# nikkolasg/playsnark

Hardware: NVIDIA B200
Metric: g1_msm_points_per_s (higher is better)
Workload: dtype u32

## Files before the change

### playsnark_b200/csrc/curve.cuh

```cuda
#pragma once
#include "field.cuh"

namespace ps {

template <bool INLINE>
struct alignas(16) Fp2T {
  Fp c0, c1;
  PS_DEV static Fp mulp(const Fp& a, const Fp& b) { if (INLINE) return a * b; else return fe_mul_call(a, b); }
  PS_DEV static Fp2T zero() { return Fp2T{Fp::zero(), Fp::zero()}; }
  PS_DEV static Fp2T one() { return Fp2T{Fp::one(), Fp::zero()}; }
  PS_DEV bool is_zero() const { return c0.is_zero() && c1.is_zero(); }
  PS_DEV bool operator==(const Fp2T& b) const { return c0 == b.c0 && c1 == b.c1; }
  PS_DEV bool operator!=(const Fp2T& b) const { return !(*this == b); }
  PS_DEV friend Fp2T operator+(const Fp2T& a, const Fp2T& b) { return Fp2T{a.c0 + b.c0, a.c1 + b.c1}; }
  PS_DEV friend Fp2T operator-(const Fp2T& a, const Fp2T& b) { return Fp2T{a.c0 - b.c0, a.c1 - b.c1}; }
  PS_DEV Fp2T neg() const { return Fp2T{c0.neg(), c1.neg()}; }
  PS_DEV Fp2T dbl() const { return Fp2T{c0.dbl(), c1.dbl()}; }
  PS_DEV friend Fp2T operator*(const Fp2T& a, const Fp2T& b) {
    Fp t0 = mulp(a.c0, b.c0);
    Fp t1 = mulp(a.c1, b.c1);
    Fp t2 = mulp(a.c0 + a.c1, b.c0 + b.c1);
    return Fp2T{t0 - t1, t2 - t0 - t1};
  }
  PS_DEV Fp2T sqr() const {
    Fp s = c0 + c1, d = c0 - c1;
    Fp m = mulp(c0, c1);
    return Fp2T{mulp(s, d), m.dbl()};
  }
};
using Fp2 = Fp2T<false>;
using Fp2I = Fp2T<true>;

PS_DEV Fp2 fp2_inv(const Fp2& a) {
  Fp d = fp_inv(fe_mul_call(a.c0, a.c0) + fe_mul_call(a.c1, a.c1));
  return Fp2{fe_mul_call(a.c0, d), fe_mul_call(a.c1, d).neg()};
}

PS_DEV Fp2 fp2_inv_serial(const Fp2& a) {
  Fp d = fp_inv_serial(fe_mul_call(a.c0, a.c0) + fe_mul_call(a.c1, a.c1));
  return Fp2{fe_mul_call(a.c0, d), fe_mul_call(a.c1, d).neg()};
}

template <class F> struct FieldInv;
template <> struct FieldInv<Fp> {
  PS_DEV static Fp inv(const Fp& a) { return fp_inv(a); }
  PS_DEV static Fp inv_serial(const Fp& a) { return fp_inv_serial(a); }
};
template <> struct FieldInv<Fp2> {
  PS_DEV static Fp2 inv(const Fp2& a) { return fp2_inv(a); }
  PS_DEV static Fp2 inv_serial(const Fp2& a) { return fp2_inv_serial(a); }
};
template <> struct FieldInv<Fp2I> {
  PS_DEV static Fp2I inv(const Fp2I& a) { Fp2 r = fp2_inv(Fp2{a.c0, a.c1}); return Fp2I{r.c0, r.c1}; }
  PS_DEV static Fp2I inv_serial(const Fp2I& a) { Fp2 r = fp2_inv_serial(Fp2{a.c0, a.c1}); return Fp2I{r.c0, r.c1}; }
};

template <class F>
struct alignas(16) Affine {
  F x, y;
  PS_DEV bool is_inf() const { return x.is_zero() && y.is_zero(); }
  PS_DEV static Affine inf() { return Affine{F::zero(), F::zero()}; }
  PS_DEV Affine neg() const { return Affine{x, y.neg()}; }
};

template <class F>
struct alignas(16) XYZZ {
  F x, y, zz, zzz;
  PS_DEV bool is_inf() const { return zz.is_zero(); }
  PS_DEV static XYZZ inf() { return XYZZ{F::zero(), F::zero(), F::zero(), F::zero()}; }
  PS_DEV static XYZZ from_affine(const Affine<F>& p) {
    if (p.is_inf()) return inf();
    return XYZZ{p.x, p.y, F::one(), F::one()};
  }
  PS_DEV XYZZ neg() const { return XYZZ{x, y.neg(), zz, zzz}; }
};

PS_DEV Fp mul_sub_pair(const Fp& a, const Fp& b, const Fp& c, const Fp& d) {
#ifndef PS_NO_LAZY_Y3
  return mul2_lazy(a, b, neg_lazy(c), d);
#else
  return a * b - c * d;
#endif
}
template <bool I>
PS_DEV Fp2T<I> mul_sub_pair(const Fp2T<I>& a, const Fp2T<I>& b, const Fp2T<I>& c, const Fp2T<I>& d) { return a * b - c * d; }

template <class F>
PS_DEV XYZZ<F> xyzz_dbl_affine(const Affine<F>& p) {
  if (p.is_inf() || p.y.is_zero()) return XYZZ<F>::inf();
  F U = p.y.dbl();
  F V = U.sqr();
  F W = U * V;
  F S = p.x * V;
  F X2 = p.x.sqr();
  F M = X2.dbl() + X2;
  F X3 = M.sqr() - S.dbl();
  F Y3 = mul_sub_pair(M, S - X3, W, p.y);
  return XYZZ<F>{X3, Y3, V, W};
}

template <class F>
PS_DEV XYZZ<F> xyzz_dbl(const XYZZ<F>& p) {
  if (p.is_inf() || p.y.is_zero()) return XYZZ<F>::inf();
  F U = p.y.dbl();
  F V = U.sqr();
  F W = U * V;
  F S = p.x * V;
  F X2 = p.x.sqr();
  F M = X2.dbl() + X2;
  F X3 = M.sqr() - S.dbl();
  F Y3 = mul_sub_pair(M, S - X3, W, p.y);
  return XYZZ<F>{X3, Y3, V * p.zz, W * p.zzz};
}

template <class F> PS_NOINLINE XYZZ<F> xyzz_dbl_c(const XYZZ<F>& p);
template <class F> PS_NOINLINE XYZZ<F> xyzz_dbl_affine_c(const Affine<F>& p);

template <class F>
PS_DEV void xyzz_madd(XYZZ<F>& acc, const Affine<F>& q) {
  if (q.is_inf()) return;
  if (acc.is_inf()) { acc = XYZZ<F>{q.x, q.y, F::one(), F::one()}; return; }
  F U2 = q.x * acc.zz;
  F S2 = q.y * acc.zzz;
  F Pd = U2 - acc.x;
  F Rd = S2 - acc.y;
  if (Pd.is_zero()) {
    if (Rd.is_zero()) acc = xyzz_dbl_affine_c(q); else acc = XYZZ<F>::inf();
    return;
  }
  F PP = Pd.sqr();
  F PPP = Pd * PP;
  F Q = acc.x * PP;
  F X3 = Rd.sqr() - PPP - Q.dbl();
  F Y3 = mul_sub_pair(Rd, Q - X3, acc.y, PPP);
  acc.x = X3;
  acc.y = Y3;
  acc.zz = acc.zz * PP;
  acc.zzz = acc.zzz * PPP;
}

template <class F>
PS_DEV void xyzz_add(XYZZ<F>& acc, const XYZZ<F>& q) {
  if (q.is_inf()) return;
  if (acc.is_inf()) { acc = q; return; }
  F U1 = acc.x * q.zz;
  F U2 = q.x * acc.zz;
  F S1 = acc.y * q.zzz;
  F S2 = q.y * acc.zzz;
  F Pd = U2 - U1;
  F Rd = S2 - S1;
  if (Pd.is_zero()) {
    if (Rd.is_zero()) acc = xyzz_dbl_c(acc); else acc = XYZZ<F>::inf();
    return;
  }
  F PP = Pd.sqr();
  F PPP = Pd * PP;
  F Q = U1 * PP;
  F X3 = Rd.sqr() - PPP - Q.dbl();
  F Y3 = mul_sub_pair(Rd, Q - X3, S1, PPP);
  acc.x = X3;
  acc.y = Y3;
  acc.zz = acc.zz * q.zz * PP;
  acc.zzz = acc.zzz * q.zzz * PPP;
}

template <class F> PS_NOINLINE XYZZ<F> xyzz_dbl_c(const XYZZ<F>& p) { return xyzz_dbl(p); }
template <class F> PS_NOINLINE XYZZ<F> xyzz_dbl_affine_c(const Affine<F>& p) { return xyzz_dbl_affine(p); }
template <class F> PS_NOINLINE void xyzz_add_c(XYZZ<F>& acc, const XYZZ<F>& q) { xyzz_add(acc, q); }
template <class F> PS_NOINLINE void xyzz_madd_c(XYZZ<F>& acc, const Affine<F>& q) { xyzz_madd(acc, q); }

template <class F>
PS_DEV Affine<F> xyzz_to_affine(const XYZZ<F>& p) {
  if (p.is_inf()) return Affine<F>::inf();
  F zzz_inv = FieldInv<F>::inv(p.zzz);
  F t = zzz_inv * p.zz;
  F zz_inv = t.sqr();
  return Affine<F>{p.x * zz_inv, p.y * zzz_inv};
}

template <class F>
PS_DEV XYZZ<F> xyzz_scalar_mul(const XYZZ<F>& p, const uint32_t* k, int nlimbs) {
  XYZZ<F> acc = XYZZ<F>::inf();
  for (int i = nlimbs - 1; i >= 0; i--) {
    uint32_t w = k[i];
#pragma unroll 1
    for (int b = 31; b >= 0; b--) {
      acc = xyzz_dbl_c(acc);
      if ((w >> b) & 1) xyzz_add_c(acc, p);
    }
  }
  return acc;
}

template <class F> PS_NOINLINE Affine<F> xyzz_to_affine_c(const XYZZ<F>& p) { return xyzz_to_affine(p); }
template <class F>
PS_NOINLINE Affine<F> xyzz_to_affine_serial(const XYZZ<F>& p) {
  if (p.is_inf()) return Affine<F>::inf();
  F zzz_inv = FieldInv<F>::inv_serial(p.zzz);
  F t = zzz_inv * p.zz;
  F zz_inv = t.sqr();
  return Affine<F>{p.x * zz_inv, p.y * zzz_inv};
}

using G1Affine = Affine<Fp>;
using G2Affine = Affine<Fp2>;
using G1XYZZ = XYZZ<Fp>;
using G2XYZZ = XYZZ<Fp2>;

}
```

### playsnark_b200/csrc/msm.cuh

```cuda
#pragma once
#include "group_ops.cuh"
#include "team.cuh"

namespace ps {

PS_DEV int msm_seg_of(const MsmPlan& p, uint32_t i) {
  int k = 0;
  while (k + 1 < p.nseg && i >= p.seg[k + 1].start) k++;
  return k;
}

struct MsmSrc {
  const uint32_t* scalars;
  uint32_t idx, b0, pt, nbase;
  int mont;
};
PS_DEV MsmSrc msm_source(const MsmPlan& p, uint32_t i) {
  MsmSrc s;
  if (p.row_len) {
    const uint32_t set = i / p.row_len;
    s.scalars = p.seg[0].scalars; s.idx = i; s.mont = (int)p.seg[0].mont;
    s.b0 = set * (uint32_t)p.S * p.D; s.nbase = p.nbase[0]; s.pt = p.toff[0] + p.seg[0].first + (i - set * p.row_len);
  } else {
    const MsmSeg sg = p.seg[msm_seg_of(p, i)];
    s.scalars = sg.scalars; s.idx = i - sg.start; s.mont = (int)sg.mont;
    s.b0 = sg.set * (uint32_t)p.S * p.D; s.nbase = p.nbase[sg.set]; s.pt = p.toff[sg.set] + sg.first + s.idx;
  }
  return s;
}

PS_DEV void msm_load_scalar(const uint32_t* scalars, uint32_t i, int mont, uint32_t k[8], bool& neg) {
  Fr x;
#pragma unroll
  for (int j = 0; j < 8; j++) x.v[j] = scalars[(size_t)i * 8 + j];
  if (mont) x = x.from_mont();
  uint32_t t = ptx_sub_cc(FrParams::HALF(0), x.v[0]);
#pragma unroll
  for (int j = 1; j < 8; j++) t = ptx_subc_cc(FrParams::HALF(j), x.v[j]);
  uint32_t borrow = ptx_subc(0, 0);
  neg = borrow != 0;
  if (neg) {
    uint32_t m[8];
    m[0] = ptx_sub_cc(FrParams::MOD(0), x.v[0]);
#pragma unroll
    for (int j = 1; j < 8; j++) m[j] = ptx_subc_cc(FrParams::MOD(j), x.v[j]);
#pragma unroll
    for (int j = 0; j < 8; j++) x.v[j] = m[j];
  }
#pragma unroll
  for (int j = 0; j < 8; j++) k[j] = x.v[j];
}

PS_DEV uint32_t msm_take_bits(uint32_t k[8], int c) {
  uint32_t v = k[0] & ((1u << c) - 1);
#pragma unroll
  for (int j = 0; j < 7; j++) k[j] = (k[j] >> c) | (k[j + 1] << (32 - c));
  k[7] >>= c;
  return v;
}

PS_DEV bool msm_next_digit(uint32_t k[8], int c, uint32_t& carry, uint32_t& mag, bool& dneg) {
  uint32_t v = msm_take_bits(k, c) + carry;
  uint32_t half = 1u << (c - 1);
  if (v > half) { mag = (1u << c) - v; dneg = true; carry = 1; }
  else { mag = v; dneg = false; carry = 0; }
  return mag != 0;
}

struct MsmCountK {
  static constexpr int BLOCK = 256;
  PS_DEV static void run(uint32_t i, MsmPlan p, uint32_t* count, uint32_t* ranks) {
    const MsmSrc src = msm_source(p, i);
    uint32_t k[8]; bool neg;
    msm_load_scalar(src.scalars, src.idx, src.mont, k, neg);
    uint32_t carry = 0;
    for (int w = 0; w < p.W; w++) {
      uint32_t mag; bool dneg;
      uint32_t rank = 0xFFFFFFFFu;
      if (msm_next_digit(k, p.c, carry, mag, dneg)) {
        uint32_t b = src.b0 + (uint32_t)(w / p.T) * p.D + (mag - 1);
        rank = ps_atomic_add(count + b, 1u);
      }
      ranks[(size_t)w * p.total + i] = rank;
    }
  }
};

struct MsmScatterK {
  static constexpr int BLOCK = 256;
  PS_DEV static void run(uint32_t i, MsmPlan p, const uint32_t* off, const uint32_t* ranks, uint32_t* ent) {
    const MsmSrc src = msm_source(p, i);
    uint32_t k[8]; bool neg;
    msm_load_scalar(src.scalars, src.idx, src.mont, k, neg);
    uint32_t carry = 0;
    for (int w = 0; w < p.W; w++) {
      uint32_t mag; bool dneg;
      if (msm_next_digit(k, p.c, carry, mag, dneg)) {
        uint32_t b = src.b0 + (uint32_t)(w / p.T) * p.D + (mag - 1);
        uint32_t pos = off[b] + ranks[(size_t)w * p.total + i];
        uint32_t idx = (uint32_t)(w % p.T) * src.nbase + src.pt;
        ent[pos] = idx | ((neg != dneg) ? 0x80000000u : 0u);
      }
    }
  }
};

PS_DEV uint32_t msm_find_bucket(const uint32_t* off, uint32_t nb, uint32_t pos) {
  uint32_t lo = 0, hi = nb;
  while (hi - lo > 1) {
    uint32_t mid = lo + (hi - lo) / 2;
    if (off[mid] <= pos) lo = mid; else hi = mid;
  }
  return lo;
}

template <class F>
PS_DEV Affine<F> msm_load_point(const Affine<F>* tab, uint32_t e) {
  Affine<F> p = tab[e & 0x7FFFFFFFu];
  if (e >> 31) p.y = p.y.neg();
  return p;
}

#ifndef PS_G1_MINB
#define PS_G1_MINB 3
#endif
#ifndef PS_G2_MINB
#define PS_G2_MINB 2
#endif
#ifndef PS_ACC_BLOCK
#define PS_ACC_BLOCK 128
#endif
template <class F>
struct MsmAccumK {
  static constexpr int BLOCK = PS_ACC_BLOCK;
  static constexpr int MIN_BLOCKS = sizeof(F) == sizeof(Fp) ? PS_G1_MINB : PS_G2_MINB;
  using Self = MsmAccumK<F>;
  PS_DEV static void run(uint32_t tid, uint32_t nb, uint32_t L, const Affine<F>* tab, const uint32_t* ent,
                         const uint32_t* off, XYZZ<F>* buckets, XYZZ<F>* slot_pt, int32_t* slot_bid,
                         uint8_t* slot_fl) {
    const uint32_t M = off[nb];
    const uint32_t head = 2 * tid, tail = 2 * tid + 1;
    slot_bid[head] = -1; slot_bid[tail] = -1;
    uint64_t p0 = (uint64_t)tid * L;
    if (p0 >= M) return;
    uint32_t cur = (uint32_t)p0;
    uint32_t end = (M - cur > L) ? cur + L : M;
    uint32_t b = msm_find_bucket(off, nb, cur);
    bool head_open = off[b] < cur;
    uint32_t bend = off[b + 1];
    XYZZ<F> acc = XYZZ<F>::inf();
    for (; cur < end; cur++) {
      if (cur == bend) {
        flush(b, acc, head_open, true, head, tail, buckets, slot_pt, slot_bid, slot_fl);
        acc = XYZZ<F>::inf();
        head_open = false;
        b++;
        while (off[b + 1] <= cur) b++;
        bend = off[b + 1];
      }
      xyzz_madd(acc, msm_load_point(tab, ent[cur]));
    }
    flush(b, acc, head_open, bend <= end, head, tail, buckets, slot_pt, slot_bid, slot_fl);
  }
  PS_DEV static void flush(uint32_t b, const XYZZ<F>& acc, bool head_open, bool closed, uint32_t head, uint32_t tail,
                           XYZZ<F>* buckets, XYZZ<F>* slot_pt, int32_t* slot_bid, uint8_t* slot_fl) {
    if (closed && !head_open) {
      buckets[b] = acc;
    } else {
      uint32_t s = head_open ? head : tail;
      slot_pt[s] = acc;
      slot_bid[s] = (int32_t)b;
      slot_fl[s] = (uint8_t)((head_open ? 1 : 0) | (closed ? 0 : 2));
    }
  }
};

template <bool T> struct Coop;
template <> struct Coop<false> {
  static constexpr uint32_t LANES = 1;
  PS_DEV explicit Coop(uint32_t&) {}
  template <class F> PS_DEV void add(XYZZ<F>& acc, const XYZZ<F>& q) const { xyzz_add_c(acc, q); }
  template <class F> PS_DEV void dbl(XYZZ<F>& p) const { p = xyzz_dbl_c(p); }
  PS_DEV bool writer() const { return true; }
  PS_DEV bool idle() const { return false; }
  PS_DEV void sync() const {}
};
template <> struct Coop<true> {
  static constexpr uint32_t LANES = TEAM;
  TeamCtx tc;
  PS_DEV explicit Coop(uint32_t& tid) : tc(TeamCtx::of(tid)) { tid >>= 2; }
  template <class F> PS_DEV void add(XYZZ<F>& acc, const XYZZ<F>& q) const { xyzz_add_t(acc, q, tc); }
  template <class F> PS_DEV void dbl(XYZZ<F>& p) const { xyzz_dbl_t(p, tc); }
  PS_DEV bool writer() const { return tc.tl == 0; }
  PS_DEV bool idle() const {
#ifdef __CUDA_ARCH__
    return false;
#else
    return tc.tl != 0;
#endif
  }
  PS_DEV void sync() const { tc.sync(); }
};

template <class F, bool T>
struct MsmRunMergeK {
  static constexpr int BLOCK = 128;
  static constexpr uint32_t RUN_MAX = 32;
  PS_DEV static void run(uint32_t t, uint32_t n_chunks, XYZZ<F>* buckets, XYZZ<F>* slot_pt, int32_t* slot_bid,
                         const uint8_t* slot_fl) {
    Coop<T> co(t);
    if (co.idle()) return;
    const uint32_t a = 2 * t + 1;
    int32_t bid = slot_bid[a];
    if (bid < 0 || slot_fl[a] != 2) return;
    uint32_t len = 0;
    for (uint32_t j = 1; j <= RUN_MAX && t + j < n_chunks; j++) {
      uint32_t h = 2 * (t + j);
      if (slot_bid[h] != bid) return;
      if (slot_fl[h] == 1) { len = j; break; }
    }
    if (!len) return;
    XYZZ<F> acc = slot_pt[a];
    for (uint32_t j = 1; j <= len; j++) co.add(acc, slot_pt[2 * (t + j)]);
    co.sync();
    if (!co.writer()) return;
    buckets[bid] = acc;
    slot_bid[a] = -1;
    for (uint32_t j = 1; j <= len; j++) slot_bid[2 * (t + j)] = -1;
  }
};

template <class F, bool T>
struct MsmCombineK {
  static constexpr int BLOCK = 128;
  PS_DEV static void flush(int32_t bid, const XYZZ<F>& acc, bool cl, bool cr, int final_pass, uint32_t tid,
                           XYZZ<F>* buckets, XYZZ<F>* out_pt, int32_t* out_bid, uint8_t* out_fl) {
    if (bid < 0) return;
    if (final_pass || (!cl && !cr)) { buckets[bid] = acc; return; }
    uint32_t s = cl ? 2 * tid : 2 * tid + 1;
    out_pt[s] = acc; out_bid[s] = bid; out_fl[s] = (uint8_t)((cl ? 1 : 0) | (cr ? 2 : 0));
  }
  PS_DEV static void run(uint32_t tid, uint32_t n_in, uint32_t f, const XYZZ<F>* in_pt, const int32_t* in_bid,
                         const uint8_t* in_fl, XYZZ<F>* buckets, XYZZ<F>* out_pt, int32_t* out_bid,
                         uint8_t* out_fl, int final_pass) {
    Coop<T> co(tid);
    if (co.idle()) return;
    const bool wr = co.writer();
    if (wr) { out_bid[2 * tid] = -1; out_bid[2 * tid + 1] = -1; }
    int32_t cur = -1; bool cl = false, cr = false;
    XYZZ<F> acc = XYZZ<F>::inf();
    for (uint32_t i = 0; i < f; i++) {
      uint64_t j = (uint64_t)tid * f + i;
      if (j >= n_in) break;
      int32_t bid = in_bid[j];
      if (bid < 0) continue;
      uint8_t fl = in_fl[j];
      if (bid != cur) {
        if (wr) flush(cur, acc, cl, cr, final_pass, tid, buckets, out_pt, out_bid, out_fl);
        cur = bid; acc = in_pt[j]; cl = fl & 1; cr = (fl & 2) != 0;
      } else {
        co.add(acc, in_pt[j]); cr = (fl & 2) != 0;
      }
    }
    if (wr) flush(cur, acc, cl, cr, final_pass, tid, buckets, out_pt, out_bid, out_fl);
  }
};

template <class F, bool T>
struct MsmReduceFirstK {
  static constexpr int BLOCK = 128;
  PS_DEV static void run(uint32_t tid, uint32_t D, uint32_t G, uint32_t g, const XYZZ<F>* buckets, XYZZ<F>* acc_out,
                         XYZZ<F>* run_out) {
    Coop<T> co(tid);
    if (co.idle()) return;
    uint32_t s = tid / G, j = tid % G;
    const XYZZ<F>* B = buckets + (size_t)s * D + (size_t)j * g;
    XYZZ<F> rr = XYZZ<F>::inf(), ww = XYZZ<F>::inf();
    for (uint32_t i = g; i-- > 0;) {
      co.add(rr, B[i]);
      co.add(ww, rr);
    }
    if (co.writer()) { acc_out[tid] = ww; run_out[tid] = rr; }
  }
};

template <class F, bool T>
struct MsmReduceK {
  static constexpr int BLOCK = 64;
  PS_DEV static void run(uint32_t tid, uint32_t n_in, uint32_t n_out, uint32_t f, int log_len, const XYZZ<F>* acc_in,
                         const XYZZ<F>* run_in, XYZZ<F>* acc_out, XYZZ<F>* run_out) {
    Coop<T> co(tid);
    if (co.idle()) return;
    uint32_t s = tid / n_out, j = tid % n_out;
    const XYZZ<F>* A = acc_in + (size_t)s * n_in + (size_t)j * f;
    const XYZZ<F>* R = run_in + (size_t)s * n_in + (size_t)j * f;
    XYZZ<F> asum = XYZZ<F>::inf(), rr = XYZZ<F>::inf(), ww = XYZZ<F>::inf();
    for (uint32_t i = f; i-- > 0;) {
      if ((size_t)j * f + i >= n_in) continue;
      co.add(asum, A[i]);
      co.add(rr, R[i]);
      if (i > 0) co.add(ww, rr);
    }
    for (int d = 0; d < log_len; d++) co.dbl(ww);
    co.add(asum, ww);
    if (co.writer()) { acc_out[tid] = asum; run_out[tid] = rr; }
  }
};

template <class F, bool T>
struct MsmBitGatherK {
  static constexpr int BLOCK = 64;
  PS_DEV static void run(uint32_t tid, uint32_t G, int g, const XYZZ<F>* acc, const XYZZ<F>* run, XYZZ<F>* Y) {
    Coop<T> co(tid);
    if (co.idle()) return;
    const uint32_t half = G / 2;
    uint32_t s = tid / ((uint32_t)(g + 1) * half), rem = tid % ((uint32_t)(g + 1) * half);
    uint32_t r = rem / half, i = rem % half;
    XYZZ<F> y;
    if (r == 0) {
      y = acc[(size_t)s * G + 2 * i];
      co.add(y, acc[(size_t)s * G + 2 * i + 1]);
    } else {
      uint32_t k = r - 1;
// ... 386 lines not shown
```

### playsnark_b200/csrc/field.cuh

```cuda
#pragma once
#include <cstdint>
#include "constants.cuh"

namespace ps {

#ifdef __CUDACC__
#define PS_NOINLINE __host__ __device__ __noinline__
#define PS_DEV __host__ __device__ __forceinline__
#else
#define PS_NOINLINE
#define PS_DEV inline
#endif

#ifdef __CUDA_ARCH__
PS_DEV uint32_t ptx_add_cc(uint32_t a, uint32_t b) { uint32_t r; asm volatile("add.cc.u32 %0,%1,%2;" : "=r"(r) : "r"(a), "r"(b)); return r; }
PS_DEV uint32_t ptx_addc_cc(uint32_t a, uint32_t b) { uint32_t r; asm volatile("addc.cc.u32 %0,%1,%2;" : "=r"(r) : "r"(a), "r"(b)); return r; }
PS_DEV uint32_t ptx_addc(uint32_t a, uint32_t b) { uint32_t r; asm volatile("addc.u32 %0,%1,%2;" : "=r"(r) : "r"(a), "r"(b)); return r; }
PS_DEV uint32_t ptx_sub_cc(uint32_t a, uint32_t b) { uint32_t r; asm volatile("sub.cc.u32 %0,%1,%2;" : "=r"(r) : "r"(a), "r"(b)); return r; }
PS_DEV uint32_t ptx_subc_cc(uint32_t a, uint32_t b) { uint32_t r; asm volatile("subc.cc.u32 %0,%1,%2;" : "=r"(r) : "r"(a), "r"(b)); return r; }
PS_DEV uint32_t ptx_subc(uint32_t a, uint32_t b) { uint32_t r; asm volatile("subc.u32 %0,%1,%2;" : "=r"(r) : "r"(a), "r"(b)); return r; }
PS_DEV void ptx_mad_wide_cc(uint32_t& lo, uint32_t& hi, uint32_t a, uint32_t b) {
  asm volatile("mad.lo.cc.u32 %0,%2,%3,%0; madc.hi.cc.u32 %1,%2,%3,%1;" : "+r"(lo), "+r"(hi) : "r"(a), "r"(b)); }
PS_DEV void ptx_madc_wide_cc(uint32_t& lo, uint32_t& hi, uint32_t a, uint32_t b) {
  asm volatile("madc.lo.cc.u32 %0,%2,%3,%0; madc.hi.cc.u32 %1,%2,%3,%1;" : "+r"(lo), "+r"(hi) : "r"(a), "r"(b)); }
PS_DEV void ptx_mul_wide(uint32_t& lo, uint32_t& hi, uint32_t a, uint32_t b) {
  asm volatile("mul.lo.u32 %0,%2,%3; mul.hi.u32 %1,%2,%3;" : "=r"(lo), "=r"(hi) : "r"(a), "r"(b)); }
#else
inline uint32_t& host_cc() { static thread_local uint32_t cc = 0; return cc; }
inline uint32_t ptx_add_cc(uint32_t a, uint32_t b) { uint64_t t = (uint64_t)a + b; host_cc() = (uint32_t)(t >> 32); return (uint32_t)t; }
inline uint32_t ptx_addc_cc(uint32_t a, uint32_t b) { uint64_t t = (uint64_t)a + b + host_cc(); host_cc() = (uint32_t)(t >> 32); return (uint32_t)t; }
inline uint32_t ptx_addc(uint32_t a, uint32_t b) { return a + b + host_cc(); }
inline uint32_t ptx_sub_cc(uint32_t a, uint32_t b) { uint64_t t = (uint64_t)a - b; host_cc() = (uint32_t)(t >> 63); return (uint32_t)t; }
inline uint32_t ptx_subc_cc(uint32_t a, uint32_t b) { uint64_t t = (uint64_t)a - b - host_cc(); host_cc() = (uint32_t)(t >> 63); return (uint32_t)t; }
inline uint32_t ptx_subc(uint32_t a, uint32_t b) { return a - b - host_cc(); }
inline void ptx_mad_wide_cc(uint32_t& lo, uint32_t& hi, uint32_t a, uint32_t b) {
  unsigned __int128 t = (unsigned __int128)a * b + (((uint64_t)hi << 32) | lo);
  lo = (uint32_t)t; hi = (uint32_t)(t >> 32); host_cc() = (uint32_t)(t >> 64); }
inline void ptx_madc_wide_cc(uint32_t& lo, uint32_t& hi, uint32_t a, uint32_t b) {
  unsigned __int128 t = (unsigned __int128)a * b + (((uint64_t)hi << 32) | lo) + host_cc();
  lo = (uint32_t)t; hi = (uint32_t)(t >> 32); host_cc() = (uint32_t)(t >> 64); }
inline void ptx_mul_wide(uint32_t& lo, uint32_t& hi, uint32_t a, uint32_t b) {
  uint64_t t = (uint64_t)a * b; lo = (uint32_t)t; hi = (uint32_t)(t >> 32); }
#endif

template <int N>
PS_DEV void mul_chain(uint32_t* acc, const uint32_t* a, uint32_t b) {
#pragma unroll
  for (int j = 0; j < N; j += 2) ptx_mul_wide(acc[j], acc[j + 1], a[j], b);
}

template <int N, bool CARRY_IN>
PS_DEV void mad_chain(uint32_t* acc, const uint32_t* a, uint32_t b) {
  if (CARRY_IN) ptx_madc_wide_cc(acc[0], acc[1], a[0], b);
  else ptx_mad_wide_cc(acc[0], acc[1], a[0], b);
#pragma unroll
  for (int j = 2; j < N; j += 2) ptx_madc_wide_cc(acc[j], acc[j + 1], a[j], b);
}

template <class P, int OFF>
PS_DEV void mad_chain_mod(uint32_t* acc, uint32_t b) {
  constexpr int N = P::N;
  ptx_mad_wide_cc(acc[0], acc[1], P::MOD(OFF), b);
#pragma unroll
  for (int j = 2; j < N; j += 2) ptx_madc_wide_cc(acc[j], acc[j + 1], P::MOD(OFF + j), b);
}

template <class P> struct Fe;
template <class P> PS_NOINLINE Fe<P> fe_mul_call(const Fe<P>& a, const Fe<P>& b);

template <class P>
struct alignas(16) Fe {
  static constexpr int N = P::N;
  using Params = P;
  uint32_t v[P::N];

  PS_DEV static Fe zero() { Fe r;
#pragma unroll
    for (int i = 0; i < N; i++) r.v[i] = 0;
    return r; }
  PS_DEV static Fe one() { Fe r;
#pragma unroll
    for (int i = 0; i < N; i++) r.v[i] = P::ONE(i);
    return r; }
  template <uint32_t (*LIMB)(int)>
  PS_DEV static Fe from_const() { Fe r;
#pragma unroll
    for (int i = 0; i < N; i++) r.v[i] = LIMB(i);
    return r; }

  PS_DEV bool is_zero() const { uint32_t o = 0;
#pragma unroll
    for (int i = 0; i < N; i++) o |= v[i];
    return o == 0; }
  PS_DEV bool operator==(const Fe& b) const { uint32_t o = 0;
#pragma unroll
    for (int i = 0; i < N; i++) o |= v[i] ^ b.v[i];
    return o == 0; }
  PS_DEV bool operator!=(const Fe& b) const { return !(*this == b); }

  PS_DEV static void final_sub(Fe& a, uint32_t top) {
    uint32_t t[N];
    t[0] = ptx_sub_cc(a.v[0], P::MOD(0));
#pragma unroll
    for (int i = 1; i < N; i++) t[i] = ptx_subc_cc(a.v[i], P::MOD(i));
    uint32_t borrow = ptx_subc(top, 0);
#pragma unroll
    for (int i = 0; i < N; i++) a.v[i] = borrow ? a.v[i] : t[i];
  }

  PS_DEV friend Fe operator+(const Fe& a, const Fe& b) {
    Fe r;
    r.v[0] = ptx_add_cc(a.v[0], b.v[0]);
#pragma unroll
    for (int i = 1; i < N; i++) r.v[i] = ptx_addc_cc(a.v[i], b.v[i]);
    uint32_t top = ptx_addc(0, 0);
    final_sub(r, top);
    return r;
  }
  PS_DEV friend Fe operator-(const Fe& a, const Fe& b) {
    Fe r;
    r.v[0] = ptx_sub_cc(a.v[0], b.v[0]);
#pragma unroll
    for (int i = 1; i < N; i++) r.v[i] = ptx_subc_cc(a.v[i], b.v[i]);
    uint32_t borrow = ptx_subc(0, 0);
    uint32_t t[N];
#pragma unroll
    for (int i = 0; i < N; i++) t[i] = P::MOD(i) & borrow;
    r.v[0] = ptx_add_cc(r.v[0], t[0]);
#pragma unroll
    for (int i = 1; i < N - 1; i++) r.v[i] = ptx_addc_cc(r.v[i], t[i]);
    r.v[N - 1] = ptx_addc(r.v[N - 1], t[N - 1]);
    return r;
  }
  PS_DEV Fe neg() const { return is_zero() ? *this : (Fe::zero() - *this); }
  PS_DEV Fe dbl() const { return *this + *this; }

  PS_DEV friend Fe operator*(const Fe& a, const Fe& b) {
    uint32_t X[N], Y[N];
    uint32_t pend;
    {
      const uint32_t bi = b.v[0];
      mul_chain<N>(X, a.v, bi);
      mul_chain<N>(Y, a.v + 1, bi);
      const uint32_t m = X[0] * P::INV;
      mad_chain_mod<P, 0>(X, m);
      uint32_t cx = ptx_addc(0, 0);
      mad_chain_mod<P, 1>(Y, m);
      pend = X[1];
#pragma unroll
      for (int k = 0; k < N - 2; k++) X[k] = X[k + 2];
      X[N - 2] = cx; X[N - 1] = 0;
    }
#pragma unroll
    for (int i = 1; i < N; i++) {
      const uint32_t bi = b.v[i];
      uint32_t* A = (i & 1) ? Y : X;
      uint32_t* S = (i & 1) ? X : Y;
      A[0] = ptx_add_cc(A[0], pend);
      mad_chain<N, true>(S, a.v + 1, bi);
      mad_chain<N, false>(A, a.v, bi);
      uint32_t cx = ptx_addc(0, 0);
      const uint32_t m = A[0] * P::INV;
      mad_chain_mod<P, 0>(A, m);
      cx = ptx_addc(cx, 0);
      mad_chain_mod<P, 1>(S, m);
      pend = A[1];
#pragma unroll
      for (int k = 0; k < N - 2; k++) A[k] = A[k + 2];
      A[N - 2] = cx; A[N - 1] = 0;
    }
    uint32_t* A = (N & 1) ? Y : X;
    uint32_t* S = (N & 1) ? X : Y;
    Fe r;
    r.v[0] = ptx_add_cc(A[0], pend);
#pragma unroll
    for (int k = 1; k < N; k++) r.v[k] = ptx_addc_cc(A[k], S[k - 1]);
    uint32_t top = ptx_addc(S[N - 1], 0);
    final_sub(r, top);
    return r;
  }
  PS_DEV Fe sqr() const { return (*this) * (*this); }


  PS_DEV Fe to_mont() const { return fe_mul_call(*this, from_const<P::R2>()); }
  PS_DEV Fe from_mont() const { Fe o = zero(); o.v[0] = 1; return fe_mul_call(*this, o); }

  PS_NOINLINE Fe pow(const uint32_t* e, int nlimbs) const {
    Fe acc = one();
    bool started = false;
    for (int i = nlimbs - 1; i >= 0; i--) {
      uint32_t w = e[i];
#pragma unroll 1
      for (int b = 31; b >= 0; b--) {
        if (started) acc = acc * acc;
        if ((w >> b) & 1) {
          if (started) acc = acc * (*this); else { acc = *this; started = true; }
        }
      }
    }
    return acc;
  }
};

template <class P, int OFF>
PS_DEV void madc_chain_mod(uint32_t* acc, uint32_t b) {
  constexpr int N = P::N;
#pragma unroll
  for (int j = 0; j < N; j += 2) ptx_madc_wide_cc(acc[j], acc[j + 1], P::MOD(OFF + j), b);
}

template <class P, bool DUAL>
PS_DEV void wide_rows(uint32_t* E, uint32_t* O, const Fe<P>& a, const Fe<P>& b, const Fe<P>& c, const Fe<P>& d) {
  constexpr int N = P::N;
#pragma unroll
  for (int k = 0; k < 2 * N + 2; k++) { E[k] = 0; O[k] = 0; }
  mul_chain<N>(E, a.v, b.v[0]);
  mul_chain<N>(O + 1, a.v + 1, b.v[0]);
  if (DUAL) {
    mad_chain<N, false>(E, c.v, d.v[0]);
    E[N] = ptx_addc(E[N], 0);
    mad_chain<N, false>(O + 1, c.v + 1, d.v[0]);
    O[N + 1] = ptx_addc(O[N + 1], 0);
  }
#pragma unroll
  for (int i = 1; i < N; i++) {
    uint32_t* ge = (i & 1) ? O : E;
    uint32_t* go = (i & 1) ? E : O;
    mad_chain<N, false>(ge + i, a.v, b.v[i]);
    ge[i + N] = ptx_addc(ge[i + N], 0);
    mad_chain<N, false>(go + i + 1, a.v + 1, b.v[i]);
    go[i + 1 + N] = ptx_addc(go[i + 1 + N], 0);
    if (DUAL) {
      mad_chain<N, false>(ge + i, c.v, d.v[i]);
      ge[i + N] = ptx_addc(ge[i + N], 0);
      mad_chain<N, false>(go + i + 1, c.v + 1, d.v[i]);
      go[i + 1 + N] = ptx_addc(go[i + 1 + N], 0);
    }
  }
}
template <int N>
PS_DEV void wide_merge(uint32_t* T, const uint32_t* E, const uint32_t* O) {
  T[0] = E[0];
  T[1] = ptx_add_cc(E[1], O[1]);
#pragma unroll
  for (int k = 2; k < 2 * N - 1; k++) T[k] = ptx_addc_cc(E[k], O[k]);
  T[2 * N - 1] = ptx_addc(E[2 * N - 1], O[2 * N - 1]);
}
template <class P>
PS_DEV void mul_wide(uint32_t* T, const Fe<P>& a, const Fe<P>& b) {
  constexpr int N = P::N;
  uint32_t E[2 * N + 2], O[2 * N + 2];
  wide_rows<P, false>(E, O, a, b, a, b);
  wide_merge<N>(T, E, O);
}
template <class P>
PS_DEV Fe<P> redc_wide(const uint32_t* T);
template <class P>
PS_DEV void mul2_wide(uint32_t* T, const Fe<P>& a, const Fe<P>& b, const Fe<P>& c, const Fe<P>& d) {
  constexpr int N = P::N;
  uint32_t E[2 * N + 2], O[2 * N + 2];
  wide_rows<P, true>(E, O, a, b, c, d);
  wide_merge<N>(T, E, O);
}
template <class P>
PS_DEV Fe<P> mul2_lazy(const Fe<P>& a, const Fe<P>& b, const Fe<P>& c, const Fe<P>& d) {
  uint32_t T[2 * P::N];
  mul2_wide(T, a, b, c, d);
  return redc_wide<P>(T);
}
template <class P>
PS_DEV Fe<P> neg_lazy(const Fe<P>& a) {
  constexpr int N = P::N;
  Fe<P> r;
  r.v[0] = ptx_sub_cc(P::MOD(0), a.v[0]);
#pragma unroll
  for (int k = 1; k < N - 1; k++) r.v[k] = ptx_subc_cc(P::MOD(k), a.v[k]);
  r.v[N - 1] = ptx_subc(P::MOD(N - 1), a.v[N - 1]);
  return r;
}

template <class P>
PS_DEV Fe<P> redc_wide(const uint32_t* T) {
  constexpr int N = P::N;
  uint32_t X[N], Y[N];
  uint32_t pend;
#pragma unroll
  for (int k = 0; k < N; k++) { X[k] = T[k]; Y[k] = 0; }
  {
    const uint32_t m = X[0] * P::INV;
    mad_chain_mod<P, 0>(X, m);
    uint32_t cx = ptx_addc(0, 0);
    mad_chain_mod<P, 1>(Y, m);
    pend = X[1];
#pragma unroll
    for (int k = 0; k < N - 2; k++) X[k] = X[k + 2];
    X[N - 2] = cx; X[N - 1] = 0;
  }
#pragma unroll
  for (int i = 1; i < N; i++) {
    uint32_t* A = (i & 1) ? Y : X;
    uint32_t* S = (i & 1) ? X : Y;
    const uint32_t m = (A[0] + pend) * P::INV;
    A[0] = ptx_add_cc(A[0], pend);
    madc_chain_mod<P, 1>(S, m);
    mad_chain_mod<P, 0>(A, m);
    uint32_t cx = ptx_addc(0, 0);
    pend = A[1];
#pragma unroll
    for (int k = 0; k < N - 2; k++) A[k] = A[k + 2];
    A[N - 2] = cx; A[N - 1] = 0;
  }
  uint32_t* A = (N & 1) ? Y : X;
  uint32_t* S = (N & 1) ? X : Y;
  Fe<P> r;
  r.v[0] = ptx_add_cc(A[0], pend);
#pragma unroll
  for (int k = 1; k < N; k++) r.v[k] = ptx_addc_cc(A[k], S[k - 1]);
  uint32_t top = ptx_addc(S[N - 1], 0);
  r.v[0] = ptx_add_cc(r.v[0], T[N]);
#pragma unroll
  for (int k = 1; k < N; k++) r.v[k] = ptx_addc_cc(r.v[k], T[N + k]);
  top = ptx_addc(top, 0);
  Fe<P>::final_sub(r, top);
  return r;
}

using Fp = Fe<FpParams>;
using Fr = Fe<FrParams>;

template <class P>
PS_DEV Fe<P> fe_ld(const Fe<P>* p) {
#ifdef __CUDA_ARCH__
  Fe<P> r;
  const uint4* q = reinterpret_cast<const uint4*>(p);
#pragma unroll
  for (int i = 0; i < P::N / 4; i++) {
    uint4 t = __ldg(q + i);
    r.v[4 * i] = t.x; r.v[4 * i + 1] = t.y; r.v[4 * i + 2] = t.z; r.v[4 * i + 3] = t.w;
  }
  return r;
#else
  return *p;
#endif
}

template <class P>
PS_NOINLINE Fe<P> fe_mul_call(const Fe<P>& a, const Fe<P>& b) { return a * b; }

}

namespace ps {
#ifdef __CUDA_ARCH__
#define PS_CEXP(name) name
#else
#define PS_CEXP(name) host_##name()
inline const uint32_t* host_c_FP_MOD_M2() { static uint32_t t[12]; for (int i = 0; i < 12; i++) t[i] = FpParams::MOD_M2(i); return t; }
inline const uint32_t* host_c_FP_SQRT_EXP() { static uint32_t t[12]; for (int i = 0; i < 12; i++) t[i] = FpParams::SQRT_EXP(i); return t; }
inline const uint32_t* host_c_FP_P_M3_D4() { static uint32_t t[12]; for (int i = 0; i < 12; i++) t[i] = FpParams::P_M3_D4(i); return t; }
inline const uint32_t* host_c_FP_P_M1_D2() { static uint32_t t[12]; for (int i = 0; i < 12; i++) t[i] = FpParams::P_M1_D2(i); return t; }
inline const uint32_t* host_c_FR_MOD_M2() { static uint32_t t[8]; for (int i = 0; i < 8; i++) t[i] = FrParams::MOD_M2(i); return t; }
#endif
template <class P>
PS_NOINLINE Fe<P> fe_inv_gcd(const Fe<P>& a) {
  constexpr int N = P::N;
  if (a.is_zero()) return a;
  uint32_t u[N], v[N], x1[N], x2[N];
#pragma unroll
  for (int i = 0; i < N; i++) { u[i] = a.v[i]; v[i] = P::MOD(i); x1[i] = 0; x2[i] = 0; }
  x1[0] = 1;
  auto halve = [](uint32_t* y, uint32_t* x) {
    constexpr int N = P::N;
#pragma unroll
    for (int i = 0; i < N - 1; i++) y[i] = (y[i] >> 1) | (y[i + 1] << 31);
    y[N - 1] >>= 1;
    uint32_t top = 0;
    if (x[0] & 1) {
      x[0] = ptx_add_cc(x[0], P::MOD(0));
#pragma unroll
      for (int i = 1; i < N; i++) x[i] = ptx_addc_cc(x[i], P::MOD(i));
      top = ptx_addc(0, 0);
    }
#pragma unroll
    for (int i = 0; i < N - 1; i++) x[i] = (x[i] >> 1) | (x[i + 1] << 31);
    x[N - 1] = (x[N - 1] >> 1) | (top << 31);
  };
  auto reduce = [](uint32_t* y, const uint32_t* z, uint32_t* x, const uint32_t* w) {
    constexpr int N = P::N;
    y[0] = ptx_sub_cc(y[0], z[0]);
#pragma unroll
    for (int i = 1; i < N - 1; i++) y[i] = ptx_subc_cc(y[i], z[i]);
    y[N - 1] = ptx_subc(y[N - 1], z[N - 1]);
    x[0] = ptx_sub_cc(x[0], w[0]);
#pragma unroll
    for (int i = 1; i < N; i++) x[i] = ptx_subc_cc(x[i], w[i]);
    uint32_t borrow = ptx_subc(0, 0);
    if (borrow) {
      x[0] = ptx_add_cc(x[0], P::MOD(0));
#pragma unroll
      for (int i = 1; i < N - 1; i++) x[i] = ptx_addc_cc(x[i], P::MOD(i));
      x[N - 1] = ptx_addc(x[N - 1], P::MOD(N - 1));
    }
  };
  auto is_one = [](const uint32_t* y) {
    constexpr int N = P::N;
    uint32_t o = y[0] ^ 1u;
#pragma unroll
    for (int i = 1; i < N; i++) o |= y[i];
    return o == 0;
  };
  auto geq = [](const uint32_t* y, const uint32_t* z) {
    constexpr int N = P::N;
    (void)ptx_sub_cc(y[0], z[0]);
#pragma unroll
    for (int i = 1; i < N; i++) (void)ptx_subc_cc(y[i], z[i]);
    return ptx_subc(0, 0) == 0;
  };
#pragma unroll 1
  for (int guard = 0; guard < 4 * 32 * N; guard++) {
    if (is_one(u) || is_one(v)) break;
#pragma unroll 1
    while ((u[0] & 1) == 0) halve(u, x1);
#pragma unroll 1
    while ((v[0] & 1) == 0) halve(v, x2);
    if (geq(u, v)) reduce(u, v, x1, x2); else reduce(v, u, x2, x1);
  }
  Fe<P> y;
  const bool from_u = is_one(u);
#pragma unroll
  for (int i = 0; i < N; i++) y.v[i] = from_u ? x1[i] : x2[i];
  const Fe<P> r2 = Fe<P>::template from_const<P::R2>();
  return y * (r2 * r2);
}
PS_DEV Fp fp_inv(const Fp& a) { return a.pow(PS_CEXP(c_FP_MOD_M2), 12); }
PS_DEV Fr fr_inv(const Fr& a) { return a.pow(PS_CEXP(c_FR_MOD_M2), 8); }
PS_DEV Fp fp_inv_serial(const Fp& a) { return fe_inv_gcd(a); }
PS_DEV Fr fr_inv_serial(const Fr& a) { return fe_inv_gcd(a); }
PS_DEV Fp fp_sqrt_candidate(const Fp& a) { return a.pow(PS_CEXP(c_FP_SQRT_EXP), 12); }
}
```

Measured before the change: 193.0 million.

## Keep G1 bucket accumulator in shared memory and raise G1 min blocks

The G1 bucket-accumulation kernel now keeps its XYZZ accumulator in a strided shared-memory slot per thread instead of in registers. A new slot-based mixed-add routine reads and writes the coordinates through load/store helpers, reordered so fewer field elements are live at once. With fewer live registers, the launch-bounds min-blocks for G1 goes from 3 to 4 to raise occupancy. The cost is extra shared-memory traffic on every add, about 24 KB of shared memory per block, and a pointer offset derived from the top limb's high bits that assumes values are fully reduced.

```diff
diff --git a/playsnark_b200/csrc/curve.cuh b/playsnark_b200/csrc/curve.cuh
--- a/playsnark_b200/csrc/curve.cuh
+++ b/playsnark_b200/csrc/curve.cuh
@@ -139,6 +139,39 @@
   acc.zzz = acc.zzz * PPP;
 }
 
+template <class F, class S>
+PS_DEV void xyzz_madd_slot(S& acc, const Affine<F>& q) {
+  if (q.is_inf()) return;
+  F U2 = acc.ld(2);
+  if (U2.is_zero()) { acc.st(0, q.x); acc.st(1, q.y); acc.st(2, F::one()); acc.st(3, F::one()); return; }
+  U2 = q.x * U2;
+  F S2 = q.y * acc.ld(3);
+  F Pd = U2 - acc.ld(0);
+  F Rd = S2 - acc.ld(1);
+  if (Pd.is_zero()) {
+    if (!Rd.is_zero() || q.y.is_zero()) { acc.st(0, F::zero()); acc.st(1, F::zero()); acc.st(2, F::zero()); acc.st(3, F::zero()); return; }
+    const F U = q.y.dbl();
+    const F X2 = q.x.sqr();
+    acc.st(1, X2.dbl() + X2);
+    acc.st(2, U.sqr());
+    acc.st(3, U * acc.ld(2));
+    acc.st(0, q.x * acc.ld(2));
+    const F M = acc.ld(1), Sx = acc.ld(0);
+    const F X3 = M.sqr() - Sx.dbl();
+    acc.st(0, X3);
+    acc.st(1, mul_sub_pair(M, Sx - X3, acc.ld(3), q.y));
+    return;
+  }
+  F PP = Pd.sqr();
+  acc.st(2, acc.ld(2) * PP);
+  F PPP = Pd * PP;
+  acc.st(3, acc.ld(3) * PPP);
+  F Q = acc.ld(0) * PP;
+  F X3 = Rd.sqr() - PPP - Q.dbl();
+  acc.st(0, X3);
+  acc.st(1, mul_sub_pair(Rd, Q - X3, acc.ld(1), PPP));
+}
+
 template <class F>
 PS_DEV void xyzz_add(XYZZ<F>& acc, const XYZZ<F>& q) {
   if (q.is_inf()) return;
diff --git a/playsnark_b200/csrc/msm.cuh b/playsnark_b200/csrc/msm.cuh
--- a/playsnark_b200/csrc/msm.cuh
+++ b/playsnark_b200/csrc/msm.cuh
@@ -122,7 +122,7 @@
 }
 
 #ifndef PS_G1_MINB
-#define PS_G1_MINB 3
+#define PS_G1_MINB 4
 #endif
 #ifndef PS_G2_MINB
 #define PS_G2_MINB 2
@@ -130,6 +130,48 @@
 #ifndef PS_ACC_BLOCK
 #define PS_ACC_BLOCK 128
 #endif
+
+template <class F>
+struct AccInRegs {
+  XYZZ<F> v;
+  PS_DEV void reset() { v = XYZZ<F>::inf(); }
+  PS_DEV void madd(const Affine<F>& q) { xyzz_madd(v, q); }
+  PS_DEV XYZZ<F> get() const { return v; }
+};
+struct AccInSmemG1 {
+  static constexpr int BLOCK = PS_ACC_BLOCK;
+#ifdef __CUDA_ARCH__
+  uint4* p;
+  PS_DEV AccInSmemG1() {
+    __shared__ uint4 sh[4 * 3 * BLOCK];
+    p = sh + threadIdx.x;
+  }
+  PS_DEV Fp ld(int k) const {
+    Fp r;
+#pragma unroll
+    for (int i = 0; i < 3; i++) {
+      const uint4 t = p[(3 * k + i) * BLOCK];
+      r.v[4 * i] = t.x; r.v[4 * i + 1] = t.y; r.v[4 * i + 2] = t.z; r.v[4 * i + 3] = t.w;
+    }
+    return r;
+  }
+  PS_DEV void st(int k, const Fp& a) {
+#pragma unroll
+    for (int i = 0; i < 3; i++) p[(3 * k + i) * BLOCK] = make_uint4(a.v[4 * i], a.v[4 * i + 1], a.v[4 * i + 2], a.v[4 * i + 3]);
+    p += a.v[11] >> 29;
+  }
+#else
+  Fp v[4];
+  PS_DEV Fp ld(int k) const { return v[k]; }
+  PS_DEV void st(int k, const Fp& a) { v[k] = a; }
+#endif
+  PS_DEV void reset() { st(0, Fp::zero()); st(1, Fp::zero()); st(2, Fp::zero()); st(3, Fp::zero()); }
+  PS_DEV void madd(const Affine<Fp>& q) { xyzz_madd_slot(*this, q); }
+  PS_DEV XYZZ<Fp> get() const { return XYZZ<Fp>{ld(0), ld(1), ld(2), ld(3)}; }
+};
+template <class F> struct AccOf { using T = AccInRegs<F>; };
+template <> struct AccOf<Fp> { using T = AccInSmemG1; };
+
 template <class F>
 struct MsmAccumK {
   static constexpr int BLOCK = PS_ACC_BLOCK;
@@ -148,19 +190,20 @@
     uint32_t b = msm_find_bucket(off, nb, cur);
     bool head_open = off[b] < cur;
     uint32_t bend = off[b + 1];
-    XYZZ<F> acc = XYZZ<F>::inf();
+    typename AccOf<F>::T acc;
+    acc.reset();
     for (; cur < end; cur++) {
       if (cur == bend) {
-        flush(b, acc, head_open, true, head, tail, buckets, slot_pt, slot_bid, slot_fl);
-        acc = XYZZ<F>::inf();
+        flush(b, acc.get(), head_open, true, head, tail, buckets, slot_pt, slot_bid, slot_fl);
+        acc.reset();
         head_open = false;
         b++;
         while (off[b + 1] <= cur) b++;
         bend = off[b + 1];
       }
-      xyzz_madd(acc, msm_load_point(tab, ent[cur]));
-    }
-    flush(b, acc, head_open, bend <= end, head, tail, buckets, slot_pt, slot_bid, slot_fl);
+      acc.madd(msm_load_point(tab, ent[cur]));
+    }
+    flush(b, acc.get(), head_open, bend <= end, head, tail, buckets, slot_pt, slot_bid, slot_fl);
   }
   PS_DEV static void flush(uint32_t b, const XYZZ<F>& acc, bool head_open, bool closed, uint32_t head, uint32_t tail,
                            XYZZ<F>* buckets, XYZZ<F>* slot_pt, int32_t* slot_bid, uint8_t* slot_fl) {
```

After: 194.4 million (median of 6 runs). About the same (+0.7%).

## Use lazy-reduced Montgomery arithmetic in G1 bucket accumulation madd

Applied to the files above, without the earlier changes.

Adds a bound-tracked lazy field type (values kept below 2p) and a variant of the Montgomery multiply and double-product reduction that skips the final conditional subtraction. The G1 bucket accumulation loop now uses a mixed add over these lazily reduced coordinates, with cheaper subtraction, zero tests modulo p, and canonicalisation only when a bucket is flushed. This removes a final_sub per multiply on the hot path, in exchange for extra zero-check comparisons and reliance on the compile-time bound asserts being correct for the BLS12-381 modulus.

```diff
diff --git a/playsnark_b200/csrc/curve.cuh b/playsnark_b200/csrc/curve.cuh
--- a/playsnark_b200/csrc/curve.cuh
+++ b/playsnark_b200/csrc/curve.cuh
@@ -169,6 +169,46 @@
 template <class F> PS_NOINLINE void xyzz_add_c(XYZZ<F>& acc, const XYZZ<F>& q) { xyzz_add(acc, q); }
 template <class F> PS_NOINLINE void xyzz_madd_c(XYZZ<F>& acc, const Affine<F>& q) { xyzz_madd(acc, q); }
 
+struct XyzzL {
+  FpK<2> x, y, zz, zzz;
+  PS_DEV static XyzzL inf() { const FpK<2> z(Fp::zero()); return XyzzL{z, z, z, z}; }
+  PS_DEV bool is_inf() const { return zz.v.is_zero(); }
+  PS_DEV XYZZ<Fp> canonical() const { return XYZZ<Fp>{ps::canonical(x), ps::canonical(y), ps::canonical(zz), ps::canonical(zzz)}; }
+};
+
+PS_DEV void xyzz_madd_lazy(XyzzL& acc, const Affine<Fp>& q, bool neg) {
+  if (q.is_inf()) return;
+  const FpK<1> qx(q.x);
+  const FpK<1> qy(neg ? neg_lazy(q.y) : q.y);
+  if (acc.is_inf()) {
+    const FpK<2> one(Fp::one());
+    acc = XyzzL{qx, qy, one, one};
+    return;
+  }
+  const FpK<2> U2 = qx * acc.zz;
+  const FpK<2> S2 = qy * acc.zzz;
+  const FpK<2> Pd = U2 - acc.x;
+  const FpK<2> Rd = S2 - acc.y;
+  if (is_zero_mod(Pd)) {
+    if (is_zero_mod(Rd)) {
+      const XYZZ<Fp> d = xyzz_dbl_affine_c(Affine<Fp>{q.x, neg ? q.y.neg() : q.y});
+      acc = XyzzL{FpK<2>(d.x), FpK<2>(d.y), FpK<2>(d.zz), FpK<2>(d.zzz)};
+    } else {
+      acc = XyzzL::inf();
+    }
+    return;
+  }
+  const FpK<2> PP = Pd * Pd;
+  const FpK<2> PPP = Pd * PP;
+  const FpK<2> Q = acc.x * PP;
+  const FpK<2> X3 = Rd * Rd - PPP - Q - Q;
+  const FpK<2> Y3 = mul2(Rd, Q - X3, neg2(acc.y), PPP);
+  acc.x = X3;
+  acc.y = Y3;
+  acc.zz = acc.zz * PP;
+  acc.zzz = acc.zzz * PPP;
+}
+
 template <class F>
 PS_DEV Affine<F> xyzz_to_affine(const XYZZ<F>& p) {
   if (p.is_inf()) return Affine<F>::inf();
diff --git a/playsnark_b200/csrc/field.cuh b/playsnark_b200/csrc/field.cuh
--- a/playsnark_b200/csrc/field.cuh
+++ b/playsnark_b200/csrc/field.cuh
@@ -135,7 +135,9 @@
   PS_DEV Fe neg() const { return is_zero() ? *this : (Fe::zero() - *this); }
   PS_DEV Fe dbl() const { return *this + *this; }
 
-  PS_DEV friend Fe operator*(const Fe& a, const Fe& b) {
+  PS_DEV friend Fe operator*(const Fe& a, const Fe& b) { return mont<true>(a, b); }
+  template <bool CANON>
+  PS_DEV static Fe mont(const Fe& a, const Fe& b) {
     uint32_t X[N], Y[N];
     uint32_t pend;
     {
@@ -174,9 +176,14 @@
     Fe r;
     r.v[0] = ptx_add_cc(A[0], pend);
 #pragma unroll
-    for (int k = 1; k < N; k++) r.v[k] = ptx_addc_cc(A[k], S[k - 1]);
-    uint32_t top = ptx_addc(S[N - 1], 0);
-    final_sub(r, top);
+    for (int k = 1; k < N - 1; k++) r.v[k] = ptx_addc_cc(A[k], S[k - 1]);
+    if (CANON) {
+      r.v[N - 1] = ptx_addc_cc(A[N - 1], S[N - 2]);
+      uint32_t top = ptx_addc(S[N - 1], 0);
+      final_sub(r, top);
+    } else {
+      r.v[N - 1] = ptx_addc(A[N - 1], S[N - 2]);
+    }
     return r;
   }
   PS_DEV Fe sqr() const { return (*this) * (*this); }
@@ -253,7 +260,7 @@
   wide_rows<P, false>(E, O, a, b, a, b);
   wide_merge<N>(T, E, O);
 }
-template <class P>
+template <class P, bool CANON = true>
 PS_DEV Fe<P> redc_wide(const uint32_t* T);
 template <class P>
 PS_DEV void mul2_wide(uint32_t* T, const Fe<P>& a, const Fe<P>& b, const Fe<P>& c, const Fe<P>& d) {
@@ -262,11 +269,11 @@
   wide_rows<P, true>(E, O, a, b, c, d);
   wide_merge<N>(T, E, O);
 }
-template <class P>
+template <class P, bool CANON = true>
 PS_DEV Fe<P> mul2_lazy(const Fe<P>& a, const Fe<P>& b, const Fe<P>& c, const Fe<P>& d) {
   uint32_t T[2 * P::N];
   mul2_wide(T, a, b, c, d);
-  return redc_wide<P>(T);
+  return redc_wide<P, CANON>(T);
 }
 template <class P>
 PS_DEV Fe<P> neg_lazy(const Fe<P>& a) {
@@ -279,7 +286,7 @@
   return r;
 }
 
-template <class P>
+template <class P, bool CANON>
 PS_DEV Fe<P> redc_wide(const uint32_t* T) {
   constexpr int N = P::N;
   uint32_t X[N], Y[N];
@@ -315,18 +322,88 @@
   Fe<P> r;
   r.v[0] = ptx_add_cc(A[0], pend);
 #pragma unroll
-  for (int k = 1; k < N; k++) r.v[k] = ptx_addc_cc(A[k], S[k - 1]);
-  uint32_t top = ptx_addc(S[N - 1], 0);
-  r.v[0] = ptx_add_cc(r.v[0], T[N]);
-#pragma unroll
-  for (int k = 1; k < N; k++) r.v[k] = ptx_addc_cc(r.v[k], T[N + k]);
-  top = ptx_addc(top, 0);
-  Fe<P>::final_sub(r, top);
+  for (int k = 1; k < N - 1; k++) r.v[k] = ptx_addc_cc(A[k], S[k - 1]);
+  if (CANON) {
+    r.v[N - 1] = ptx_addc_cc(A[N - 1], S[N - 2]);
+    uint32_t top = ptx_addc(S[N - 1], 0);
+    r.v[0] = ptx_add_cc(r.v[0], T[N]);
+#pragma unroll
+    for (int k = 1; k < N; k++) r.v[k] = ptx_addc_cc(r.v[k], T[N + k]);
+    top = ptx_addc(top, 0);
+    Fe<P>::final_sub(r, top);
+  } else {
+    r.v[N - 1] = ptx_addc(A[N - 1], S[N - 2]);
+    r.v[0] = ptx_add_cc(r.v[0], T[N]);
+#pragma unroll
+    for (int k = 1; k < N - 1; k++) r.v[k] = ptx_addc_cc(r.v[k], T[N + k]);
+    r.v[N - 1] = ptx_addc(r.v[N - 1], T[2 * N - 1]);
+  }
   return r;
 }
 
 using Fp = Fe<FpParams>;
 using Fr = Fe<FrParams>;
+
+template <int K>
+struct FpK {
+  static_assert(K >= 1 && K <= 8, "FpK: the product needs (K + 1) p < R");
+  Fp v;
+  FpK() = default;
+  PS_DEV explicit FpK(const Fp& a) : v(a) {}
+  template <int J>
+  PS_DEV FpK(const FpK<J>& a) : v(a.v) { static_assert(J <= K, "FpK: a bound only widens"); }
+};
+template <int A, int B>
+PS_DEV FpK<2> operator*(const FpK<A>& a, const FpK<B>& b) {
+  static_assert(A * B <= 9, "FpK product: a b / R + p must stay below 2p");
+  return FpK<2>(Fp::mont<false>(a.v, b.v));
+}
+template <int A, int B, int C, int D>
+PS_DEV FpK<2> mul2(const FpK<A>& a, const FpK<B>& b, const FpK<C>& c, const FpK<D>& d) {
+  static_assert(A * B + C * D <= 9, "FpK mul2: (a b + c d) / R + p must stay below 2p");
+  return FpK<2>(mul2_lazy<FpParams, false>(a.v, b.v, c.v, d.v));
+}
+PS_DEV constexpr uint32_t fp_2p_limb(int i) { return (FpParams::MOD(i) << 1) | (i ? FpParams::MOD(i - 1) >> 31 : 0u); }
+template <int A, int B>
+PS_DEV FpK<2> operator-(const FpK<A>& a, const FpK<B>& b) {
+  static_assert(A <= 2 && B <= 2, "FpK difference: operands up to 2p");
+  constexpr int N = Fp::N;
+  Fp r;
+  r.v[0] = ptx_sub_cc(a.v.v[0], b.v.v[0]);
+#pragma unroll
+  for (int i = 1; i < N; i++) r.v[i] = ptx_subc_cc(a.v.v[i], b.v.v[i]);
+  const uint32_t borrow = ptx_subc(0, 0);
+  r.v[0] = ptx_add_cc(r.v[0], fp_2p_limb(0) & borrow);
+#pragma unroll
+  for (int i = 1; i < N - 1; i++) r.v[i] = ptx_addc_cc(r.v[i], fp_2p_limb(i) & borrow);
+  r.v[N - 1] = ptx_addc(r.v[N - 1], fp_2p_limb(N - 1) & borrow);
+  return FpK<2>(r);
+}
+template <int B>
+PS_DEV FpK<2> neg2(const FpK<B>& b) {
+  static_assert(B <= 2, "FpK negation: operand up to 2p");
+  constexpr int N = Fp::N;
+  Fp r;
+  r.v[0] = ptx_sub_cc(fp_2p_limb(0), b.v.v[0]);
+#pragma unroll
+  for (int i = 1; i < N - 1; i++) r.v[i] = ptx_subc_cc(fp_2p_limb(i), b.v.v[i]);
+  r.v[N - 1] = ptx_subc(fp_2p_limb(N - 1), b.v.v[N - 1]);
+  return FpK<2>(r);
+}
+PS_DEV bool is_zero_mod(const FpK<2>& a) {
+  const uint32_t lo = a.v.v[0];
+  if (lo != 0 && lo != FpParams::MOD(0) && lo != fp_2p_limb(0)) return false;
+  uint32_t z = 0, zp = 0, z2p = 0;
+#pragma unroll
+  for (int i = 0; i < Fp::N; i++) { z |= a.v.v[i]; zp |= a.v.v[i] ^ FpParams::MOD(i); z2p |= a.v.v[i] ^ fp_2p_limb(i); }
+  return z == 0 || zp == 0 || z2p == 0;
+}
+PS_DEV Fp canonical(const FpK<2>& a) {
+  Fp r = a.v;
+  Fp::final_sub(r, 0);
+  Fp::final_sub(r, 0);
+  return r;
+}
 
 template <class P>
 PS_DEV Fe<P> fe_ld(const Fe<P>* p) {
diff --git a/playsnark_b200/csrc/msm.cuh b/playsnark_b200/csrc/msm.cuh
--- a/playsnark_b200/csrc/msm.cuh
+++ b/playsnark_b200/csrc/msm.cuh
@@ -120,6 +120,22 @@
   if (e >> 31) p.y = p.y.neg();
   return p;
 }
+
+template <class F>
+struct MsmAcc {
+  using T = XYZZ<F>;
+  PS_DEV static void add(T& acc, const Affine<F>* tab, uint32_t e) { xyzz_madd(acc, msm_load_point(tab, e)); }
+  PS_DEV static XYZZ<F> out(const T& acc) { return acc; }
+};
+template <>
+struct MsmAcc<Fp> {
+  using T = XyzzL;
+  PS_DEV static void add(T& acc, const Affine<Fp>* tab, uint32_t e) {
+    const Affine<Fp>* q = tab + (e & 0x7FFFFFFFu);
+    xyzz_madd_lazy(acc, Affine<Fp>{fe_ld(&q->x), fe_ld(&q->y)}, e >> 31);
+  }
+  PS_DEV static XYZZ<Fp> out(const T& acc) { return acc.canonical(); }
+};
 
 #ifndef PS_G1_MINB
 #define PS_G1_MINB 3
@@ -148,27 +164,28 @@
     uint32_t b = msm_find_bucket(off, nb, cur);
     bool head_open = off[b] < cur;
     uint32_t bend = off[b + 1];
-    XYZZ<F> acc = XYZZ<F>::inf();
+    typename MsmAcc<F>::T acc = MsmAcc<F>::T::inf();
     for (; cur < end; cur++) {
       if (cur == bend) {
         flush(b, acc, head_open, true, head, tail, buckets, slot_pt, slot_bid, slot_fl);
-        acc = XYZZ<F>::inf();
+        acc = MsmAcc<F>::T::inf();
         head_open = false;
         b++;
         while (off[b + 1] <= cur) b++;
         bend = off[b + 1];
       }
-      xyzz_madd(acc, msm_load_point(tab, ent[cur]));
+      MsmAcc<F>::add(acc, tab, ent[cur]);
     }
     flush(b, acc, head_open, bend <= end, head, tail, buckets, slot_pt, slot_bid, slot_fl);
   }
-  PS_DEV static void flush(uint32_t b, const XYZZ<F>& acc, bool head_open, bool closed, uint32_t head, uint32_t tail,
+  PS_DEV static void flush(uint32_t b, const typename MsmAcc<F>::T& acc, bool head_open, bool closed, uint32_t head, uint32_t tail,
                            XYZZ<F>* buckets, XYZZ<F>* slot_pt, int32_t* slot_bid, uint8_t* slot_fl) {
+    const XYZZ<F> o = MsmAcc<F>::out(acc);
     if (closed && !head_open) {
-      buckets[b] = acc;
+      buckets[b] = o;
     } else {
       uint32_t s = head_open ? head : tail;
-      slot_pt[s] = acc;
+      slot_pt[s] = o;
       slot_bid[s] = (int32_t)b;
       slot_fl[s] = (uint8_t)((head_open ? 1 : 0) | (closed ? 0 : 2));
     }
```

After: 192.9 million before, 181.0 million after, median of 6. 6.2% lower.
